# KKKSQJ/DeepLearning

Measured on NVIDIA H100. Metric: images/sec (ResNet-50 training step), higher is better.
Workload: dtype bf16

## Files before the change

deeplearning_b200/csrc/abi_conv.cu:

```cuda
#include <string.h>
#include "../../include/b200cls.h"
#include "conv_gemm.cuh"
#include "conv1x1_stream.cuh"
#include "conv_tap64.cuh"
#include "host_utils.h"
#include "wgrad_gemm.cuh"

using namespace b200;

namespace {

constexpr uint32_t kFwdDescLbo = 16, kFwdDescSbo = 1024;
constexpr uint32_t kWgDescLbo = 8192, kWgDescSbo = 1024, kWgDescKstep = 2048;

struct Box3 {
  int b1, b2, b3;
};

Box3 choose_box(long long d1, long long d2, long long d3, int P) {
  Box3 best{P, 1, 1};
  double best_cost = -1;
  for (int b1 = 1; b1 <= P; b1 <<= 1) {
    for (int b2 = 1; b1 * b2 <= P; b2 <<= 1) {
      const int b3 = P / (b1 * b2);
// ... 29 lines not shown
};

View make_view(const void* base, int B, int H, int W, int C, int s, int ph, int pw) {
  View v;
  v.base = static_cast<const char*>(base) + (static_cast<long long>(ph) * W + pw) * C * 2;
  v.dims[0] = C;
  v.dims[1] = (W - pw + s - 1) / s;
  v.dims[2] = (H - ph + s - 1) / s;
  v.dims[3] = B;
  v.strides[0] = 1;
  v.strides[1] = static_cast<uint64_t>(s) * C;
  v.strides[2] = static_cast<uint64_t>(s) * W * C;
  v.strides[3] = static_cast<uint64_t>(H) * W * C;
  return v;
}
View make_flat_view(const void* base, long long M, int C) {
  View v;
  v.base = base;
  v.dims[0] = C;
  v.dims[1] = M;
  v.dims[2] = 1;
  v.dims[3] = 1;
  v.strides[0] = 1;
  v.strides[1] = C;
  v.strides[2] = static_cast<uint64_t>(M) * C;
  v.strides[3] = static_cast<uint64_t>(M) * C;
  return v;
}
View act_view(const void* base, int B, int H, int W, int C, bool flat) {
  return flat ? make_flat_view(base, static_cast<long long>(B) * H * W, C) : make_view(base, B, H, W, C, 1, 0, 0);
}
int encode_view(CUtensorMap* m, const View& v, const Box3& bx) {
  uint32_t box[4] = {64, (uint32_t)bx.b1, (uint32_t)bx.b2, (uint32_t)bx.b3};
  if (v.dims[1] == 0 || v.dims[2] == 0 || v.dims[3] == 0) {
    set_error("empty activation view");
    return EINVAL_;
  }
  return encode_tmap_bf16(m, v.base, 4, v.dims, v.strides, box);
}

int encode_matrix(CUtensorMap* m, const void* base, long long cols, long long rows, int box_rows) {
  uint64_t dims[2] = {static_cast<uint64_t>(cols), static_cast<uint64_t>(rows)};
  uint64_t strides[2] = {1, static_cast<uint64_t>(cols)};
  uint32_t box[2] = {64, static_cast<uint32_t>(box_rows)};
  return encode_tmap_bf16(m, base, 2, dims, strides, box);
}

template <class Params>
int encode_taps(Params& p, CUtensorMap (&maps)[4], const void* x, int B, int H, int W, int C, int ksize, int stride,
                const Box3& bx) {
  int rc;
  if (stride == 1) {
    if ((rc = encode_view(&maps[0], act_view(x, B, H, W, C, ksize == 1), bx))) return rc;
    for (int i = 1; i < 4; ++i) maps[i] = maps[0];
  } else {
    for (int ph = 0; ph < 2; ++ph)
      for (int pw = 0; pw < 2; ++pw)
        if ((rc = encode_view(&maps[ph * 2 + pw], make_view(x, B, H, W, C, 2, ph, pw), bx))) return rc;
  }
  const int pad = pad_of(ksize);
  for (int kh = 0; kh < ksize; ++kh)
    for (int kw = 0; kw < ksize; ++kw) {
      const int t = kh * ksize + kw, dh = kh - pad, dw = kw - pad;
      const int ph = stride == 2 ? dh & 1 : 0, pw = stride == 2 ? dw & 1 : 0;
      p.tap_map[t] = static_cast<int8_t>(ph * 2 + pw);
      p.tap_o1[t] = static_cast<int8_t>((dw - pw) / stride);
      p.tap_o2[t] = static_cast<int8_t>((dh - ph) / stride);
    }
  return OK;
}

void quarter_box(const Box3& bx, Box3* qb, int (&o1)[4], int (&o2)[4], int (&o3)[4]) {
  for (int q = 0; q < 4; ++q) o1[q] = o2[q] = o3[q] = 0;
  if (bx.b3 >= 4) {
    *qb = Box3{bx.b1, bx.b2, bx.b3 / 4};
    for (int q = 0; q < 4; ++q) o3[q] = q * (bx.b3 / 4);
  } else if (bx.b3 == 2) {
    *qb = Box3{bx.b1, bx.b2 / 2, 1};
    if (bx.b2 >= 2) {
      for (int q = 0; q < 4; ++q) {
        o2[q] = (q & 1) * (bx.b2 / 2);
        o3[q] = q >> 1;
      }
    } else {
      *qb = Box3{bx.b1 / 2, 1, 1};
      for (int q = 0; q < 4; ++q) {
        o1[q] = (q & 1) * (bx.b1 / 2);
        o3[q] = q >> 1;
      }
    }
  } else if (bx.b2 >= 4) {
    *qb = Box3{bx.b1, bx.b2 / 4, 1};
    for (int q = 0; q < 4; ++q) o2[q] = q * (bx.b2 / 4);
  } else if (bx.b2 == 2) {
    *qb = Box3{bx.b1 / 2, 1, 1};
    for (int q = 0; q < 4; ++q) {
      o1[q] = (q & 1) * (bx.b1 / 2);
      o2[q] = q >> 1;
    }
  } else {
    *qb = Box3{bx.b1 / 4, 1, 1};
    for (int q = 0; q < 4; ++q) o1[q] = q * (bx.b1 / 4);
  }
}

int setup_output(ConvGemmParams& p, const View& dv, int N, int out_f32, const View* auxv) {
  const long long d1 = dv.dims[1], d2 = dv.dims[2], d3 = dv.dims[3];
  const Box3 bx = choose_box(d1, d2, d3, 128);
  p.box1 = bx.b1, p.box2 = bx.b2, p.box3 = bx.b3;
  p.dim1 = static_cast<int>(d1), p.dim2 = static_cast<int>(d2), p.dim3 = static_cast<int>(d3);
  p.tiles1 = static_cast<int>((d1 + bx.b1 - 1) / bx.b1);
  p.tiles2 = static_cast<int>((d2 + bx.b2 - 1) / bx.b2);
  p.tiles3 = static_cast<int>((d3 + bx.b3 - 1) / bx.b3);
  p.N = N;
  const int BN = N <= 64 ? 64 : 128;
  p.n_tiles = (N + BN - 1) / BN;
  Box3 qb;
  quarter_box(bx, &qb, p.qoff1, p.qoff2, p.qoff3);
  p.out_f32 = out_f32;
  if (dv.base != nullptr) {
    uint32_t box[4] = {out_f32 ? 32u : 64u, (uint32_t)qb.b1, (uint32_t)qb.b2, (uint32_t)qb.b3};
    int rc = out_f32 ? encode_tmap_f32(&p.d_map, dv.base, 4, dv.dims, dv.strides, box)
                     : encode_tmap_bf16(&p.d_map, dv.base, 4, dv.dims, dv.strides, box);
    if (rc) return rc;
  }
  p.has_aux_out = 0;
  if (auxv != nullptr) {
    uint32_t box[4] = {64u, (uint32_t)qb.b1, (uint32_t)qb.b2, (uint32_t)qb.b3};
    int rc = encode_tmap_bf16(&p.aux_map, auxv->base, 4, auxv->dims, auxv->strides, box);
    if (rc) return rc;
    p.has_aux_out = 1;
  }
  return OK;
}
Box3 box_of(const ConvGemmParams& p) { return Box3{p.box1, p.box2, p.box3}; }

bool bn_mask_complete(const b200_bn_mask_t* m) { return m->x_raw && m->scale && m->shift && m->stats; }
void set_bn_mask(ConvGemmParams& p, const b200_bn_mask_t* m, const View& dv) {
  p.mask_in = static_cast<const __nv_bfloat16*>(m->x_raw);
  p.ms1 = static_cast<long long>(dv.strides[1]);
  p.ms2 = static_cast<long long>(dv.strides[2]);
  p.ms3 = static_cast<long long>(dv.strides[3]);
  p.bn_scale = m->scale, p.bn_shift = m->shift, p.stats = m->stats;
}

int conv_grid(int tiles, int n_tiles, bool stats) {
  int grid = tiles < device_sm_count() ? tiles : device_sm_count();
  if (stats) grid = grid / n_tiles * n_tiles;
  return grid;
}

template <int BLOCK_N, int EPI>
int launch_conv_gemm_epi(const ConvGemmParams& q, int grid, cudaStream_t st) {
  using Cfg = ConvGemmCfg<BLOCK_N>;
  static bool configured = false;
  if (!configured) {
    B200_CHECK_CUDA(cudaFuncSetAttribute(conv_gemm_kernel<BLOCK_N, EPI>, cudaFuncAttributeMaxDynamicSharedMemorySize,
                                         Cfg::SMEM_BYTES));
    configured = true;
  }
  B200_CHECK_CUDA(launch_pdl(conv_gemm_kernel<BLOCK_N, EPI>, dim3(grid), dim3(Cfg::THREADS), Cfg::SMEM_BYTES, st, q));
  B200_LAUNCHED();
  return OK;
}

int epilogue_flags(const ConvGemmParams& p) {
  int f = 0;
  if (p.bias) f |= kEpiBias;
  if (p.colscale) f |= kEpiColscale;
  f |= (p.act & 3) << kEpiActShift;
  if (p.residual) f |= p.res_f32 ? kEpiResF32 : kEpiResBf16;
  if (p.has_aux_out) f |= kEpiAux;
  if (p.out_f32) f |= kEpiOutF32;
  if (p.out_direct) f |= kEpiDirect;
  if (p.stats) f |= kEpiStats;
  if (p.rowscale) f |= kEpiRowscale;
  if (p.affine) f = (f & ~(kEpiBias | kEpiColscale)) | kEpiAffine;
  if (p.mask_in) f |= p.bn_scale ? kEpiBnMask : kEpiMask;
  if (p.bn_scale) f &= ~kEpiStats;
  return f;
}

#define B200_EPI_LIST(X)                                                                                  \
  X(kEpiStats)                                              \
  X(0)                                                      \
  X(kEpiResBf16)                                            \
  X(kEpiBias)                                               \
  X(kEpiBias | kEpiResF32 | kEpiOutF32)                     \
  X(kEpiBias | kEpiColscale | kEpiResF32 | kEpiOutF32)      \
  X(kEpiBias | (2 << kEpiActShift) | kEpiAux)               \
  X(3 << kEpiActShift)                                      \
  X((3 << kEpiActShift) | kEpiStats)                        \
  X(kEpiOutF32)                                             \
  X(kEpiBias | kEpiOutF32)                                  \
  X(kEpiAffine | kEpiResBf16 | (1 << kEpiActShift))        \
  X(kEpiAffine | (1 << kEpiActShift))                      \
  X(kEpiAffine)                                            \
  X(kEpiMask | kEpiResBf16 | kEpiStats)                    \
  X(kEpiBnMask)                                            \
  X(kEpiBnMask | kEpiBias)

bool tap64_ok(const ConvGemmParams& p) {
  const int f = epilogue_flags(p);
  return p.N == 64 && p.n_tiles == 1 && p.k_per_tap == 64 && p.k_blocks_per_tap == 1 && !p.var_taps && !p.chan_window &&
         p.num_taps >= 2 && p.num_taps <= 9 && (f == 0 || f == kEpiStats) && p.dim1 % p.box1 == 0 && p.dim2 % p.box2 == 0 &&
         p.dim3 % p.box3 == 0;
}
template <bool kStats>
int launch_tap64(const ConvGemmParams& q, int grid, cudaStream_t st) {
  static bool configured = false;
  if (!configured) {
    B200_CHECK_CUDA(cudaFuncSetAttribute(conv_tap64_kernel<kStats>, cudaFuncAttributeMaxDynamicSharedMemorySize, kTap64SmemBytes));
    configured = true;
  }
  B200_CHECK_CUDA(launch_pdl(conv_tap64_kernel<kStats>, dim3(grid), dim3(384), kTap64SmemBytes, st, q));
  B200_LAUNCHED();
  return OK;
}

template <int BLOCK_N>
int launch_conv_gemm(const ConvGemmParams& p, cudaStream_t st) {
  const int tiles = p.tiles1 * p.tiles2 * p.tiles3 * p.n_tiles;
  const int grid = conv_grid(tiles, p.n_tiles, p.stats != nullptr);
  B200_REQUIRE(grid > 0, "conv_gemm: %d channel blocks exceed the SM count (BN statistics need grid %% n_tiles == 0)", p.n_tiles);
  ConvGemmParams q = p;
  q.desc_lbo = kFwdDescLbo;
  q.desc_sbo = kFwdDescSbo;
  if constexpr (BLOCK_N == 64) {
    if (tap64_ok(p)) return p.stats != nullptr ? launch_tap64<true>(q, grid, st) : launch_tap64<false>(q, grid, st);
  }
  switch (epilogue_flags(p)) {
#define B200_EPI_CASE(F) \
  case (F):              \
    return launch_conv_gemm_epi<BLOCK_N, (F)>(q, grid, st);
    B200_EPI_LIST(B200_EPI_CASE)
#undef B200_EPI_CASE
    default:
      return launch_conv_gemm_epi<BLOCK_N, kEpiGeneric>(q, grid, st);
  }
}


bool stream_ok(long long pixels, int K, int N) {
  return (K == 64 || K == 128 || K == 256) && N % 256 == 0 && pixels % 128 == 0 && pixels / 128 < (1LL << 30);
}
int stream_grid(long long pixels, int N) {
  const int n_tiles = N / 256;
  const long long items = pixels / 128 * n_tiles;
  int grid = items < device_sm_count() ? static_cast<int>(items) : device_sm_count();
  return grid / n_tiles * n_tiles;
}

template <int KB, int MODE>
int launch_stream(const StreamParams& q, int grid, cudaStream_t st) {
  using Cfg = StreamCfg<KB, MODE>;
  static bool configured = false;
  if (!configured) {
    B200_CHECK_CUDA(cudaFuncSetAttribute(conv1x1_stream_kernel<KB, MODE>, cudaFuncAttributeMaxDynamicSharedMemorySize,
                                         Cfg::SMEM_BYTES));
    configured = true;
  }
  B200_CHECK_CUDA(launch_pdl(conv1x1_stream_kernel<KB, MODE>, dim3(grid), dim3(Cfg::THREADS), Cfg::SMEM_BYTES, st, q));
  B200_LAUNCHED();
  return OK;
}

int run_stream(int mode, const void* a, const void* w, void* out, const void* res, const void* mask, const float* scale,
               const float* shift, float* stats, long long pixels, int K, int N, cudaStream_t st) {
  StreamParams q;
  memset(&q, 0, sizeof(q));
  int rc;
  if ((rc = encode_matrix(&q.a_map, a, K, pixels, 128))) return rc;
  if ((rc = encode_matrix(&q.b_map, w, K, N, 256))) return rc;
  if ((rc = encode_matrix(&q.out_map, out, N, pixels, 16))) return rc;
  if (res != nullptr && (rc = encode_matrix(&q.res_map, res, N, pixels, 16))) return rc;
  if (mask != nullptr && (rc = encode_matrix(&q.mask_map, mask, N, pixels, 16))) return rc;
  q.m_tiles = static_cast<int>(pixels / 128);
  q.n_tiles = N / 256;
  q.N = N;
  q.scale = scale, q.shift = shift, q.stats = stats;
  const int grid = stream_grid(pixels, N);
  if (mode == kStreamAffine)
    return K == 64 ? launch_stream<1, kStreamAffine>(q, grid, st)
                   : (K == 128 ? launch_stream<2, kStreamAffine>(q, grid, st) : launch_stream<4, kStreamAffine>(q, grid, st));
  if (mode == kStreamBnRelu)
    return K == 64 ? launch_stream<1, kStreamBnRelu>(q, grid, st)
                   : (K == 128 ? launch_stream<2, kStreamBnRelu>(q, grid, st) : launch_stream<4, kStreamBnRelu>(q, grid, st));
  return K == 64 ? launch_stream<1, kStreamMask>(q, grid, st)
                 : (K == 128 ? launch_stream<2, kStreamMask>(q, grid, st) : launch_stream<4, kStreamMask>(q, grid, st));
}

int dispatch_conv_gemm(ConvGemmParams& p, int N, cudaStream_t st) {
  if (N <= 64) return launch_conv_gemm<64>(p, st);
  return launch_conv_gemm<128>(p, st);
}
int block_n_for(int N) { return N <= 64 ? 64 : 128; }

template <int BLOCK_NG, bool kGrouped = false>
int launch_wgrad(const WgradParams& p, cudaStream_t st) {
  using Cfg = WgradCfg<BLOCK_NG>;
  static bool configured = false;
  if (!configured) {
    if constexpr (kGrouped) {
      B200_CHECK_CUDA(cudaFuncSetAttribute(wgrad_gemm_kernel<BLOCK_NG, false, true>,
                                           cudaFuncAttributeMaxDynamicSharedMemorySize, Cfg::SMEM_BYTES));
    } else {
      B200_CHECK_CUDA(cudaFuncSetAttribute(wgrad_gemm_kernel<BLOCK_NG, false>, cudaFuncAttributeMaxDynamicSharedMemorySize,
// ... 601 lines not shown
```

deeplearning_b200/csrc/conv_gemm.cuh:

```cuda
#pragma once
#include <cstdio>
#include "common.cuh"

namespace b200 {

constexpr int kMaxTaps = 16;

struct alignas(64) ConvGemmParams {
  CUtensorMap a_maps[4];
  CUtensorMap b_map;
  CUtensorMap d_map;
  CUtensorMap aux_map;
  int num_taps;
  int k_per_tap;
  int k_blocks_per_tap;
  int tiles1, tiles2, tiles3;
  int box1, box2, box3;
  int dim1, dim2, dim3;
  int qoff1[4], qoff2[4], qoff3[4];
  int n_tiles;
  int N;
  int8_t tap_map[kMaxTaps];
  int8_t tap_o1[kMaxTaps];
  int8_t tap_o2[kMaxTaps];
  int8_t tap_w[kMaxTaps];
  float* stats;
  const float* bias;
  const float* colscale;
  int act;
  int out_f32;
  int res_f32;
  int has_aux_out;
  const void* residual;
  long long rs1, rs2, rs3;
  const __nv_bfloat16* aux_in;
  long long as1, as2, as3;
  uint32_t desc_lbo, desc_sbo;
  float* out_direct;
  long long ld_out;
  const float* rowscale;
  int rows_per_sample;
  int var_taps;
  int kb_total;
  int16_t tap_kb[kMaxTaps];
  int32_t tap_k0[kMaxTaps];
  const __nv_bfloat16* mask_in;
  long long ms1, ms2, ms3;
  int affine;
  const float* bn_scale;
  const float* bn_shift;
  int chan_window;
};

template <int BLOCK_N>
struct ConvGemmCfg {
  static constexpr int BLOCK_M = 128;
  static constexpr int BLOCK_K = 64;
  static constexpr int A_BYTES = BLOCK_M * BLOCK_K * 2;
  static constexpr int B_BYTES = BLOCK_N * BLOCK_K * 2;
  static constexpr int STAGES = BLOCK_N == 128 ? 4 : 5;
  static constexpr int STAGE_BYTES = A_BYTES + B_BYTES;
  static constexpr int EPI_WARPS = 4;
  static constexpr int SLAB_BYTES = 32 * 128;
  static constexpr int STAGING_BYTES = EPI_WARPS * 2 * SLAB_BYTES;
  static constexpr int IMG_BYTES = BLOCK_M * BLOCK_N * 4;
  static constexpr int IMGS = BLOCK_N == 128 ? 1 : 2;
  static constexpr int BAR_BYTES = 256;
  static constexpr int SMEM_BYTES = STAGES * STAGE_BYTES + STAGING_BYTES + IMGS * IMG_BYTES + BAR_BYTES + 1024;
  static constexpr int THREADS = 512;
  static_assert(SMEM_BYTES <= 227 * 1024, "shared memory of one H100 block");
  static_assert(2 * STAGES + 2 * IMGS <= BAR_BYTES / 8, "mbarriers");
};

__device__ __forceinline__ void gelu_parts(float x, float& tail, float& e) {
  const float az = fabsf(x) * 0.70710678118654752f;
  float t;
  asm("rcp.approx.ftz.f32 %0, %1;" : "=f"(t) : "f"(fmaf(0.3275911f, az, 1.0f)));
  float poly = fmaf(1.061405429f, t, -1.453152027f);
  poly = fmaf(poly, t, 1.421413741f);
  poly = fmaf(poly, t, -0.284496736f);
  poly = fmaf(poly, t, 0.254829592f);
  asm("ex2.approx.ftz.f32 %0, %1;" : "=f"(e) : "f"(-1.4426950408889634f * az * az));
  tail = 0.5f * poly * t * e;
}
__device__ __forceinline__ float gelu_erf(float x) {
  float tail, e;
  gelu_parts(x, tail, e);
  return x * (x >= 0.f ? 1.0f - tail : tail);
}
__device__ __forceinline__ float gelu_erf_grad(float x) {
  float tail, e;
  gelu_parts(x, tail, e);
  const float cdf = x >= 0.f ? 1.0f - tail : tail;
  return fmaf(x * 0.3989422804014327f, e, cdf);
}

__device__ __forceinline__ void gelu_parts2(float x0, float x1, uint64_t& cdf, uint64_t& e) {
  const uint64_t az = f2_pack(fabsf(x0) * 0.70710678118654752f, fabsf(x1) * 0.70710678118654752f);
  float d0, d1, t0, t1, g0, g1, e0, e1, h0, h1;
  f2_unpack(f2_fma(f2_bcast(0.3275911f), az, f2_bcast(1.0f)), d0, d1);
  asm("rcp.approx.ftz.f32 %0, %1;" : "=f"(t0) : "f"(d0));
  asm("rcp.approx.ftz.f32 %0, %1;" : "=f"(t1) : "f"(d1));
  const uint64_t t = f2_pack(t0, t1);
  uint64_t poly = f2_fma(f2_bcast(1.061405429f), t, f2_bcast(-1.453152027f));
  poly = f2_fma(poly, t, f2_bcast(1.421413741f));
  poly = f2_fma(poly, t, f2_bcast(-0.284496736f));
  poly = f2_fma(poly, t, f2_bcast(0.254829592f));
  f2_unpack(f2_mul(f2_mul(az, az), f2_bcast(-1.4426950408889634f)), g0, g1);
  asm("ex2.approx.ftz.f32 %0, %1;" : "=f"(e0) : "f"(g0));
  asm("ex2.approx.ftz.f32 %0, %1;" : "=f"(e1) : "f"(g1));
  e = f2_pack(e0, e1);
  f2_unpack(f2_fma(f2_mul(f2_mul(poly, t), e), f2_bcast(-0.5f), f2_bcast(0.5f)), h0, h1);
  cdf = f2_add(f2_pack(copysignf(h0, x0), copysignf(h1, x1)), f2_bcast(0.5f));
}
__device__ __forceinline__ void gelu_erf2(float& x0, float& x1) {
  uint64_t cdf, e;
  gelu_parts2(x0, x1, cdf, e);
  f2_unpack(f2_mul(f2_pack(x0, x1), cdf), x0, x1);
}
__device__ __forceinline__ void gelu_erf_val_grad2(float& x0, float& x1, float& g0, float& g1) {
  uint64_t cdf, e;
  gelu_parts2(x0, x1, cdf, e);
  const uint64_t x = f2_pack(x0, x1);
  f2_unpack(f2_fma(f2_mul(x, f2_bcast(0.3989422804014327f)), e, cdf), g0, g1);
  f2_unpack(f2_mul(x, cdf), x0, x1);
}

#ifdef CONV_PROFILE
#define CPROF_DECL(N) long long cp_t[N] = {}; long long cp_0 = clock64(), cp_1;
#define CPROF_TICK(i) { cp_1 = clock64(); cp_t[i] += cp_1 - cp_0; cp_0 = cp_1; }
#else
#define CPROF_DECL(N)
#define CPROF_TICK(i)
#endif

template <int S>
__device__ __forceinline__ void butterfly_step(float (&px)[32], int lane) {
  const bool up = (lane & S) != 0;
#pragma unroll
  for (int i = 0; i < S; ++i) {
    const float send = up ? px[i] : px[i + S];
    const float keep = up ? px[i + S] : px[i];
    px[i] = keep + __shfl_xor_sync(0xffffffffu, send, S);
  }
}

constexpr int kEpiGeneric = -1;
constexpr int kEpiBias = 1, kEpiColscale = 2, kEpiActShift = 2 , kEpiResBf16 = 16, kEpiResF32 = 32,
              kEpiAux = 64, kEpiOutF32 = 128, kEpiDirect = 256, kEpiStats = 512,
              kEpiRowscale = 1024 ,
              kEpiAffine = 2048, kEpiMask = 4096, kEpiBnMask = 8192;

template <int BLOCK_N, int EPI = kEpiGeneric>
__global__ void __launch_bounds__(512, 1) conv_gemm_kernel(const __grid_constant__ ConvGemmParams p) {
  static_assert(BLOCK_N == 64 || BLOCK_N == 128, "64- or 128-column tiles");
  using Cfg = ConvGemmCfg<BLOCK_N>;
  constexpr int STAGES = Cfg::STAGES;
  constexpr int IMGS = Cfg::IMGS;
  extern __shared__ uint8_t smem_raw[];
  uint8_t* smem = reinterpret_cast<uint8_t*>((reinterpret_cast<uintptr_t>(smem_raw) + 1023) & ~uintptr_t(1023));
  uint8_t* stage_base = smem;
  uint8_t* staging = smem + STAGES * Cfg::STAGE_BYTES;
  uint8_t* img = staging + Cfg::STAGING_BYTES;
  uint64_t* bars = reinterpret_cast<uint64_t*>(img + IMGS * Cfg::IMG_BYTES);
  uint64_t* full_bar = bars;
  uint64_t* empty_bar = bars + STAGES;
  uint64_t* img_full = bars + 2 * STAGES;
  uint64_t* img_empty = bars + 2 * STAGES + IMGS;

  const int warp_idx = threadIdx.x >> 5;
  const int lane = threadIdx.x & 31;
  const int m_tiles = p.tiles1 * p.tiles2 * p.tiles3;
  const int num_tiles = m_tiles * p.n_tiles;
  const int num_kb = p.var_taps ? p.kb_total : p.num_taps * p.k_blocks_per_tap;

  if (warp_idx == 0 && lane == 0) {
    for (int i = 0; i < 4; ++i) tma_prefetch_desc(&p.a_maps[i]);
    tma_prefetch_desc(&p.b_map);
    tma_prefetch_desc(&p.d_map);
    for (int i = 0; i < STAGES; ++i) {
      mbar_init(&full_bar[i], 1);
      mbar_init(&empty_bar[i], 2);
    }
    for (int i = 0; i < IMGS; ++i) {
      mbar_init(&img_full[i], 8);
      mbar_init(&img_empty[i], Cfg::EPI_WARPS);
    }
    fence_mbar_init();
  }
  __syncthreads();
  pdl_wait();

  if (warp_idx < 4) {
    setmaxnreg_dec<40>();
    if (warp_idx == 0 && lane == 0) {
      int stage = 0;
      uint32_t phase = 0;
      CPROF_DECL(2)
      for (int tile = blockIdx.x; tile < num_tiles; tile += gridDim.x) {
        const int n_tile = tile % p.n_tiles;
        const int m_tile = tile / p.n_tiles;
        const int t1 = m_tile % p.tiles1;
        const int t2 = (m_tile / p.tiles1) % p.tiles2;
        const int t3 = m_tile / (p.tiles1 * p.tiles2);
        const int c1 = t1 * p.box1, c2 = t2 * p.box2, c3 = t3 * p.box3;
        int tap = 0, cb = 0;
        int kb_in_tap = p.var_taps ? p.tap_kb[0] : p.k_blocks_per_tap;
        for (int kb = 0; kb < num_kb; ++kb, ++cb) {
          if (cb == kb_in_tap) {
            cb = 0;
            ++tap;
            if (p.var_taps) kb_in_tap = p.tap_kb[tap];
          }
          const int wk = p.var_taps ? p.tap_k0[tap] + cb * 64 : p.tap_w[tap] * p.k_per_tap + cb * 64;
          CPROF_TICK(1)
          mbar_wait_backoff(&empty_bar[stage], phase ^ 1);
          CPROF_TICK(0)
          uint8_t* a_dst = stage_base + stage * Cfg::STAGE_BYTES;
          uint8_t* b_dst = a_dst + Cfg::A_BYTES;
          mbar_expect_tx(&full_bar[stage], Cfg::STAGE_BYTES);
          tma_load_4d(a_dst, &p.a_maps[p.tap_map[tap]], &full_bar[stage], p.chan_window ? n_tile * BLOCK_N : cb * 64, c1 + p.tap_o1[tap],
                      c2 + p.tap_o2[tap], c3);
          tma_load_2d(b_dst, &p.b_map, &full_bar[stage], wk, n_tile * BLOCK_N);
          if (++stage == STAGES) {
            stage = 0;
            phase ^= 1;
          }
        }
      }
#ifdef CONV_PROFILE
      if (blockIdx.x == 0) {
        const int nt = (num_tiles - 1) / gridDim.x + 1;
        printf("conv producer: wait_empty %lld issue %lld  (cycles/tile, %d tiles, %d k-blocks)\n", cp_t[0] / nt, cp_t[1] / nt, nt, num_kb);
      }
#endif
    }
  } else if (warp_idx < 12) {
    setmaxnreg_dec<112>();
    const int wg = (warp_idx - 4) >> 2;
    const uint64_t desc_a0 = make_smem_desc_sw128(smem_u32(stage_base) + wg * 8192, p.desc_lbo, p.desc_sbo);
    const uint64_t desc_b0 = make_smem_desc_sw128(smem_u32(stage_base) + Cfg::A_BYTES, p.desc_lbo, p.desc_sbo);
    int stage = 0;
    uint32_t phase = 0;
    int it = 0;
    CPROF_DECL(3)
    for (int tile = blockIdx.x; tile < num_tiles; tile += gridDim.x, ++it) {
      float acc[BLOCK_N / 2];
#pragma unroll
      for (int i = 0; i < BLOCK_N / 2; ++i) acc[i] = 0.f;
      int prev = -1;
      CPROF_TICK(2)
      for (int kb = 0; kb < num_kb; ++kb) {
        mbar_wait(&full_bar[stage], phase);
        wgmma_fence();
        const uint64_t soff = static_cast<uint64_t>(stage) * (Cfg::STAGE_BYTES >> 4);
        const uint64_t da = desc_a0 + soff, db = desc_b0 + soff;
#pragma unroll
        for (int k = 0; k < 4; ++k) Wgmma<BLOCK_N, 0, 0>::mma(acc, da + 2 * k, db + 2 * k, 1u);
        wgmma_commit();
        wgmma_wait<1>();
        if (prev >= 0 && (threadIdx.x & 127) == 0) mbar_arrive(&empty_bar[prev]);
        prev = stage;
        if (++stage == STAGES) {
          stage = 0;
          phase ^= 1;
        }
      }
      wgmma_wait<0>();
      wgmma_reg_fence(acc);
      if ((threadIdx.x & 127) == 0) mbar_arrive(&empty_bar[prev]);
      CPROF_TICK(0)
      const int b = IMGS == 1 ? 0 : it % IMGS;
      mbar_wait(&img_empty[b], ((it / IMGS) & 1) ^ 1);
      CPROF_TICK(1)
      acc_to_img<BLOCK_N>(acc, smem_u32(img + b * Cfg::IMG_BYTES), BLOCK_N, 64 * wg, 0);
      __syncwarp();
      if (lane == 0) mbar_arrive(&img_full[b]);
    }
#ifdef CONV_PROFILE
    if (blockIdx.x == 0 && lane == 0 && (warp_idx & 3) == 0) {
      const int nt = (num_tiles - 1) / gridDim.x + 1;
      printf("conv mma wg %d: main loop %lld wait img_empty %lld acc->img %lld  (cycles/tile)\n", wg, cp_t[0] / nt, cp_t[1] / nt,
             cp_t[2] / nt);
    }
#endif
  } else {
    setmaxnreg_inc<248>();
    const int q = warp_idx - 12;
    const int row = q * 32 + lane;
    const uint32_t stage_s = smem_u32(staging + q * 2 * Cfg::SLAB_BYTES);
    const uint32_t row_s = lane * 128;
    const uint32_t sw = (lane & 7) << 4;
    uint32_t stat_off[8];
#pragma unroll
    for (int m = 0; m < 8; ++m) stat_off[m] = m * 128 + ((((lane >> 2) ^ m) << 4) | ((lane & 3) << 2));
    constexpr bool G = EPI < 0;
    constexpr bool kAffine = !G && (EPI & kEpiAffine) != 0;
    constexpr bool kBnMask = !G && (EPI & kEpiBnMask) != 0;
    constexpr bool kMask = !G && (EPI & (kEpiMask | kEpiBnMask)) != 0;
    const int N = p.N;
    const float* const bias = (!kAffine && (G || (EPI & kEpiBias))) ? p.bias : nullptr;
    const float* const colscale = (!kAffine && (G || (EPI & kEpiColscale))) ? p.colscale : nullptr;
    const int act_bits = G ? p.act : ((EPI >> kEpiActShift) & 3);
    const int act = kAffine ? 0 : act_bits;
    const bool has_res = G ? (p.residual != nullptr) : ((EPI & (kEpiResBf16 | kEpiResF32)) != 0);
    const bool res_f32 = G ? (p.res_f32 != 0) : ((EPI & kEpiResF32) != 0);
    const bool has_aux = G ? (p.has_aux_out != 0) : ((EPI & kEpiAux) != 0);
    const bool out_f32 = G ? (p.out_f32 != 0) : ((EPI & kEpiOutF32) != 0);
    float* const out_direct = (G || (EPI & kEpiDirect)) ? p.out_direct : nullptr;
    float* const stats = (G || (EPI & (kEpiStats | kEpiBnMask))) ? p.stats : nullptr;
    const float* const rowscale = G ? p.rowscale : nullptr;
    const bool need_rowmap = has_res || act == 3 || kMask || out_direct != nullptr || rowscale != nullptr || p.dim1 % p.box1 != 0 ||
                             p.dim2 % p.box2 != 0 || p.dim3 % p.box3 != 0;
    const bool full_cols = (N % BLOCK_N) == 0;
    uint32_t store_counter = 0;
    const int unit_cols = out_f32 ? 32 : 64;
    const int units = BLOCK_N / unit_cols;
    const int nsub = out_f32 ? 1 : 2;
    constexpr int SLOTS = 2;
    uint64_t run_s[SLOTS], run_q[SLOTS];
    float run_x[SLOTS][2];
#pragma unroll
    for (int k = 0; k < SLOTS; ++k) run_s[k] = 0, run_q[k] = 0, run_x[k][0] = run_x[k][1] = 0.f;
    int it = 0;
    CPROF_DECL(2)
    for (int tile = blockIdx.x; tile < num_tiles; tile += gridDim.x, ++it) {
      const int b = IMGS == 1 ? 0 : it % IMGS;
      const uint32_t img_s = smem_u32(img + b * Cfg::IMG_BYTES);
      const int n_tile = tile % p.n_tiles;
      const int m_tile = tile / p.n_tiles;
      const int t1 = m_tile % p.tiles1;
      const int t2 = (m_tile / p.tiles1) % p.tiles2;
      const int t3 = m_tile / (p.tiles1 * p.tiles2);
      const int c1 = t1 * p.box1, c2 = t2 * p.box2, c3 = t3 * p.box3;
      int p1 = 0, p2 = 0, p3 = 0;
      bool row_ok = true;
      if (need_rowmap) {
        const int i1 = row % p.box1;
        const int i2 = (row / p.box1) % p.box2;
        const int i3 = row / (p.box1 * p.box2);
        p1 = c1 + i1, p2 = c2 + i2, p3 = c3 + i3;
        row_ok = (p1 < p.dim1) && (p2 < p.dim2) && (p3 < p.dim3);
      }
      const int s1 = c1 + p.qoff1[q], s2 = c2 + p.qoff2[q], s3 = c3 + p.qoff3[q];

      uint4 nx_b[4];
      float4 nx_f[8];
      uint4 nx_m[4];
      auto issue_pre = [&](int u, int h) {
        const int ncp = n_tile * BLOCK_N + u * unit_cols + h * 32;
        if (n_tile * BLOCK_N + u * unit_cols >= N || !row_ok) return;
        if (has_res) {
          const long long off = p3 * p.rs3 + p2 * p.rs2 + p1 * p.rs1 + ncp;
          if (res_f32) {
            const float4* rp = reinterpret_cast<const float4*>(static_cast<const float*>(p.residual) + off);
#pragma unroll
            for (int j = 0; j < 8; ++j)
              if (full_cols || ncp + j * 4 < N) nx_f[j] = __ldg(rp + j);
          } else {
            const uint4* rp = reinterpret_cast<const uint4*>(static_cast<const __nv_bfloat16*>(p.residual) + off);
#pragma unroll
            for (int j = 0; j < 4; ++j)
              if (full_cols || ncp + j * 8 < N) nx_b[j] = __ldg(rp + j);
          }
        }
        if (act == 3) {
          const uint4* ap = reinterpret_cast<const uint4*>(p.aux_in + p3 * p.as3 + p2 * p.as2 + p1 * p.as1 + ncp);
#pragma unroll
          for (int j = 0; j < 4; ++j)
            if (full_cols || ncp + j * 8 < N) nx_b[j] = __ldg(ap + j);
        }
        if constexpr (kMask) {
          const uint4* mp = reinterpret_cast<const uint4*>(p.mask_in + p3 * p.ms3 + p2 * p.ms2 + p1 * p.ms1 + ncp);
#pragma unroll
          for (int j = 0; j < 4; ++j)
            if (full_cols || ncp + j * 8 < N) nx_m[j] = __ldg(mp + j);
        }
      };
      if (has_res || act == 3 || kMask) issue_pre(0, 0);
      CPROF_TICK(1)
      mbar_wait(&img_full[b], (it / IMGS) & 1);
      CPROF_TICK(0)

#pragma unroll 1
      for (int u = 0; u < units; ++u) {
        const int n0 = n_tile * BLOCK_N + u * unit_cols;
        const bool chunk_live = n0 < N;
        const uint32_t buf_s = stage_s + (store_counter & 1) * Cfg::SLAB_BYTES;
        const uint32_t aux_s = stage_s + ((store_counter + 1) & 1) * Cfg::SLAB_BYTES;
        if (chunk_live && out_direct == nullptr) {
          if (lane == 0) {
            if (has_aux) tma_store_wait_read<0>(); else tma_store_wait_read<1>();
          }
          __syncwarp();
        }
#pragma unroll 1
        for (int h = 0; h < nsub; ++h) {
          uint32_t v[32];
          img_ld32(img_s, BLOCK_N, row, u * unit_cols + h * 32, v);
          if (u == units - 1 && h == nsub - 1) {
            __syncwarp();
            if (lane == 0) mbar_arrive(&img_empty[b]);
          }
          uint4 pre_b[4];
          float4 pre_f[8];
          uint4 pre_m[4];
          if (has_res || act == 3 || kMask) {
#pragma unroll
            for (int j = 0; j < 4; ++j) pre_b[j] = nx_b[j];
#pragma unroll
            for (int j = 0; j < 8; ++j) pre_f[j] = nx_f[j];
            if constexpr (kMask) {
#pragma unroll
              for (int j = 0; j < 4; ++j) pre_m[j] = nx_m[j];
            }
            if (h + 1 < nsub)
              issue_pre(u, h + 1);
            else if (u + 1 < units)
              issue_pre(u + 1, 0);
          }
          if (!chunk_live) continue;
          const int nc = n0 + h * 32;
          float f[32];
#pragma unroll
          for (int j = 0; j < 32; ++j) f[j] = __uint_as_float(v[j]);
          if constexpr (kAffine) {
#pragma unroll
            for (int j = 0; j < 8; ++j) {
              const float4 s4 = __ldg(reinterpret_cast<const float4*>(p.colscale + nc) + j);
              const float4 b4 = __ldg(reinterpret_cast<const float4*>(p.bias + nc) + j);
              f2_unpack(f2_fma(f2_pack(f[j * 4 + 0], f[j * 4 + 1]), f2_pack(s4.x, s4.y), f2_pack(b4.x, b4.y)), f[j * 4 + 0], f[j * 4 + 1]);
              f2_unpack(f2_fma(f2_pack(f[j * 4 + 2], f[j * 4 + 3]), f2_pack(s4.z, s4.w), f2_pack(b4.z, b4.w)), f[j * 4 + 2], f[j * 4 + 3]);
            }
          }
          if (bias != nullptr) {
            if (full_cols) {
#pragma unroll
              for (int j = 0; j < 8; ++j) {
                const float4 b4 = __ldg(reinterpret_cast<const float4*>(bias + nc) + j);
                f2_unpack(f2_add(f2_pack(f[j * 4 + 0], f[j * 4 + 1]), f2_pack(b4.x, b4.y)), f[j * 4 + 0], f[j * 4 + 1]);
                f2_unpack(f2_add(f2_pack(f[j * 4 + 2], f[j * 4 + 3]), f2_pack(b4.z, b4.w)), f[j * 4 + 2], f[j * 4 + 3]);
              }
            } else {
#pragma unroll
              for (int j = 0; j < 32; ++j) f[j] += (nc + j < N) ? __ldg(bias + nc + j) : 0.0f;
            }
          }
          if (has_aux) {
            const uint32_t z = row_ok ? 0xffffffffu : 0u;
            if (act == 2) {
#pragma unroll
              for (int j = 0; j < 4; ++j) {
                float g[8];
#pragma unroll
                for (int i = 0; i < 8; i += 2) gelu_erf_val_grad2(f[j * 8 + i], f[j * 8 + i + 1], g[i], g[i + 1]);
                sts128(aux_s + row_s + ((((h * 4 + j) << 4)) ^ sw), pack_bf16x2(g[0], g[1]) & z, pack_bf16x2(g[2], g[3]) & z,
                       pack_bf16x2(g[4], g[5]) & z, pack_bf16x2(g[6], g[7]) & z);
              }
            } else {
#pragma unroll
              for (int j = 0; j < 4; ++j)
                sts128(aux_s + row_s + ((((h * 4 + j) << 4)) ^ sw), pack_bf16x2(f[j * 8 + 0], f[j * 8 + 1]) & z,
                       pack_bf16x2(f[j * 8 + 2], f[j * 8 + 3]) & z, pack_bf16x2(f[j * 8 + 4], f[j * 8 + 5]) & z,
                       pack_bf16x2(f[j * 8 + 6], f[j * 8 + 7]) & z);
            }
          }
          if (act == 1) {
#pragma unroll
            for (int j = 0; j < 32; ++j) f[j] = fmaxf(f[j], 0.0f);
          } else if (act == 2) {
            if (!has_aux) {
#pragma unroll
              for (int j = 0; j < 32; j += 2) gelu_erf2(f[j], f[j + 1]);
            }
          } else if (act == 3 && row_ok) {
#pragma unroll
            for (int j = 0; j < 4; ++j) {
              if (full_cols || nc + j * 8 < N) {
                float a[8];
                unpack8(pre_b[j], a);
#pragma unroll
                for (int i = 0; i < 8; i += 2)
                  f2_unpack(f2_mul(f2_pack(f[j * 8 + i], f[j * 8 + i + 1]), f2_pack(a[i], a[i + 1])), f[j * 8 + i],
                            f[j * 8 + i + 1]);
              }
            }
          }
          if (colscale != nullptr) {
#pragma unroll
            for (int j = 0; j < 32; ++j) f[j] *= (full_cols || nc + j < N) ? __ldg(colscale + nc + j) : 0.0f;
          }
          if (rowscale != nullptr && row_ok) {
            const long long pix = (static_cast<long long>(p3) * p.dim2 + p2) * p.dim1 + p1;
            const float rs = __ldg(rowscale + pix / p.rows_per_sample);
#pragma unroll
            for (int j = 0; j < 32; ++j) f[j] *= rs;
          }
          if (has_res && row_ok) {
            if (res_f32) {
#pragma unroll
              for (int j = 0; j < 8; ++j) {
                if (full_cols || nc + j * 4 < N) {
                  const float4 r = pre_f[j];
                  f2_unpack(f2_add(f2_pack(f[j * 4 + 0], f[j * 4 + 1]), f2_pack(r.x, r.y)), f[j * 4 + 0], f[j * 4 + 1]);
                  f2_unpack(f2_add(f2_pack(f[j * 4 + 2], f[j * 4 + 3]), f2_pack(r.z, r.w)), f[j * 4 + 2], f[j * 4 + 3]);
                }
              }
            } else {
#pragma unroll
              for (int j = 0; j < 4; ++j) {
                if (full_cols || nc + j * 8 < N) {
                  float r[8];
                  unpack8(pre_b[j], r);
#pragma unroll
                  for (int i = 0; i < 8; i += 2)
                    f2_unpack(f2_add(f2_pack(f[j * 8 + i], f[j * 8 + i + 1]), f2_pack(r[i], r[i + 1])), f[j * 8 + i],
                              f[j * 8 + i + 1]);
                }
              }
            }
          }
          if constexpr (kAffine) {
            if (act_bits == 1) {
#pragma unroll
              for (int j = 0; j < 32; ++j) f[j] = fmaxf(f[j], 0.0f);
            }
          }
          if constexpr (kBnMask) {
            float px[32];
            if (row_ok) {
#pragma unroll
              for (int j = 0; j < 4; ++j) {
                float x8[8];
                unpack8(pre_m[j], x8);
#pragma unroll
                for (int i = 0; i < 8; ++i) px[j * 8 + i] = x8[i];
              }
#pragma unroll
              for (int j = 0; j < 8; ++j) {
                const float4 s4 = __ldg(reinterpret_cast<const float4*>(p.bn_scale + nc) + j);
                const float4 b4 = __ldg(reinterpret_cast<const float4*>(p.bn_shift + nc) + j);
                const float sc4[4] = {s4.x, s4.y, s4.z, s4.w}, sh4[4] = {b4.x, b4.y, b4.z, b4.w};
#pragma unroll
                for (int i = 0; i < 4; ++i) {
                  const float fm =
                      fmaf(px[j * 4 + i], sc4[i], sh4[i]) > 0.f ? __bfloat162float(__float2bfloat16_rn(f[j * 4 + i])) : 0.f;
                  f[j * 4 + i] = fm;
                  px[j * 4 + i] *= fm;
                }
              }
            } else {
#pragma unroll
              for (int j = 0; j < 32; ++j) px[j] = 0.f;
            }
            butterfly_step<16>(px, lane);
            butterfly_step<8>(px, lane);
            butterfly_step<4>(px, lane);
            butterfly_step<2>(px, lane);
            butterfly_step<1>(px, lane);
            const int slot = units == 1 ? (it & 1) : u;
#pragma unroll
            for (int k = 0; k < SLOTS; ++k) {
              if (k == slot) {
                run_x[k][0] += h == 0 ? px[0] : 0.f;
                run_x[k][1] += h == 0 ? 0.f : px[0];
              }
            }
          } else if constexpr (kMask) {
            if (row_ok) {
#pragma unroll
              for (int j = 0; j < 4; ++j) {
                const uint32_t w[4] = {pre_m[j].x, pre_m[j].y, pre_m[j].z, pre_m[j].w};
#pragma unroll
                for (int i = 0; i < 4; ++i) {
                  if ((w[i] & 0x7fffu) == 0u) f[j * 8 + 2 * i] = 0.f;
                  if ((w[i] & 0x7fff0000u) == 0u) f[j * 8 + 2 * i + 1] = 0.f;
                }
              }
            }
          }
          if (out_direct != nullptr) {
            if (row_ok) {
              const long long pix = (static_cast<long long>(p3) * p.dim2 + p2) * p.dim1 + p1;
              float* op = out_direct + pix * p.ld_out + nc;
#pragma unroll
              for (int j = 0; j < 32; ++j)
                if (nc + j < N) op[j] = f[j];
            }
            continue;
          }
          if (!row_ok) {
#pragma unroll
            for (int j = 0; j < 32; ++j) f[j] = 0.f;
          }
          if (out_f32) {
#pragma unroll
            for (int j = 0; j < 8; ++j)
              sts128(buf_s + row_s + ((j << 4) ^ sw), __float_as_uint(f[j * 4 + 0]), __float_as_uint(f[j * 4 + 1]),
                     __float_as_uint(f[j * 4 + 2]), __float_as_uint(f[j * 4 + 3]));
          } else {
#pragma unroll
            for (int j = 0; j < 4; ++j)
              sts128(buf_s + row_s + (((h * 4 + j) << 4) ^ sw), pack_bf16x2(f[j * 8 + 0], f[j * 8 + 1]),
                     pack_bf16x2(f[j * 8 + 2], f[j * 8 + 3]), pack_bf16x2(f[j * 8 + 4], f[j * 8 + 5]),
                     pack_bf16x2(f[j * 8 + 6], f[j * 8 + 7]));
          }
        }
        if (!chunk_live || out_direct != nullptr) continue;
        __syncwarp();
        if (stats != nullptr) {
          uint64_t a_s = 0, a_q = 0;
#pragma unroll
          for (int r = 0; r < 32; ++r) {
            const uint32_t w = lds32(buf_s + (r >> 3) * 1024 + stat_off[r & 7]);
            const uint64_t x2 = f2_pack(bf16_lo(w), bf16_hi(w));
            a_s = f2_add(a_s, x2);
            a_q = f2_fma(x2, x2, a_q);
          }
          const int slot = units == 1 ? (it & 1) : u;
#pragma unroll
          for (int k = 0; k < SLOTS; ++k) {
            if (k == slot) {
              run_s[k] = f2_add(run_s[k], a_s);
              run_q[k] = f2_add(run_q[k], a_q);
            }
          }
        }
        fence_proxy_async_smem();
        __syncwarp();
        if (lane == 0) {
          asm volatile("cp.async.bulk.tensor.4d.global.shared::cta.bulk_group [%0, {%2, %3, %4, %5}], [%1];" ::"l"(
                           reinterpret_cast<uint64_t>(&p.d_map)),
                       "r"(buf_s), "r"(n0), "r"(s1), "r"(s2), "r"(s3)
                       : "memory");
          tma_store_commit();
          if (has_aux) {
            asm volatile("cp.async.bulk.tensor.4d.global.shared::cta.bulk_group [%0, {%2, %3, %4, %5}], [%1];" ::"l"(
                             reinterpret_cast<uint64_t>(&p.aux_map)),
                         "r"(aux_s), "r"(n0), "r"(s1), "r"(s2), "r"(s3)
                         : "memory");
            tma_store_commit();
          }
        }
        store_counter += has_aux ? 2 : 1;
      }
    }
#ifdef CONV_PROFILE
    if (blockIdx.x == 0 && lane == 0 && q == 0) {
      const int nt = (num_tiles - 1) / gridDim.x + 1;
      printf("conv epilogue: wait img_full %lld drain %lld  (cycles/tile)\n", cp_t[0] / nt, cp_t[1] / nt);
    }
#endif
    if (stats != nullptr) {
      const int cta = static_cast<int>(blockIdx.x);
      const int n_tile = cta % p.n_tiles;
      const int grp = cta / p.n_tiles;
#pragma unroll
      for (int k = 0; k < SLOTS; ++k) {
        const int srow = units == 1 ? (grp * 4 + q) * 2 + k : grp * 4 + q;
        const int col = n_tile * BLOCK_N + (units == 1 ? 0 : k * unit_cols) + 2 * lane;
        if (col < N) {
          float s_lo, s_hi, q_lo, q_hi;
          f2_unpack(run_s[k], s_lo, s_hi);
          f2_unpack(run_q[k], q_lo, q_hi);
          float* sp = stats + static_cast<long long>(srow) * 2 * N + col;
          *reinterpret_cast<float2*>(sp) = make_float2(s_lo, s_hi);
          if constexpr (kBnMask) {
            sp += N - lane;
            sp[0] = run_x[k][0];
            sp[32] = run_x[k][1];
          } else {
            *reinterpret_cast<float2*>(sp + N) = make_float2(q_lo, q_hi);
          }
        }
      }
    }
    if (lane == 0) tma_store_wait_all<0>();
  }
}

}
```

Measured before the change: 8800.

## Add second epilogue warpgroup for BLOCK_N=64 and BN-mask conv GEMM kernels

Makes the conv GEMM config depend on the epilogue variant and adds a second epilogue warpgroup for 64-column tiles and BN-mask epilogues. The two groups either alternate tiles or split the columns of a single accumulator image. Register budgets per role are rebalanced with setmaxnreg, and stage counts drop to fit staging memory. The BN-mask path now keeps scale/shift in lanes and shuffles them, moves the product reduction after the store, and recomputes stats offsets to save registers. The aim is to stop the epilogue from bottlenecking the MMA pipeline, at the cost of fewer pipeline stages and tighter register limits per role.

```diff
diff --git a/deeplearning_b200/csrc/abi_conv.cu b/deeplearning_b200/csrc/abi_conv.cu
--- a/deeplearning_b200/csrc/abi_conv.cu
+++ b/deeplearning_b200/csrc/abi_conv.cu
@@ -205,7 +205,7 @@
 
 template <int BLOCK_N, int EPI>
 int launch_conv_gemm_epi(const ConvGemmParams& q, int grid, cudaStream_t st) {
-  using Cfg = ConvGemmCfg<BLOCK_N>;
+  using Cfg = ConvGemmCfg<BLOCK_N, EPI>;
   static bool configured = false;
   if (!configured) {
     B200_CHECK_CUDA(cudaFuncSetAttribute(conv_gemm_kernel<BLOCK_N, EPI>, cudaFuncAttributeMaxDynamicSharedMemorySize,
diff --git a/deeplearning_b200/csrc/conv_gemm.cuh b/deeplearning_b200/csrc/conv_gemm.cuh
--- a/deeplearning_b200/csrc/conv_gemm.cuh
+++ b/deeplearning_b200/csrc/conv_gemm.cuh
@@ -52,26 +52,6 @@
   int chan_window;
 };
 
-template <int BLOCK_N>
-struct ConvGemmCfg {
-  static constexpr int BLOCK_M = 128;
-  static constexpr int BLOCK_K = 64;
-  static constexpr int A_BYTES = BLOCK_M * BLOCK_K * 2;
-  static constexpr int B_BYTES = BLOCK_N * BLOCK_K * 2;
-  static constexpr int STAGES = BLOCK_N == 128 ? 4 : 5;
-  static constexpr int STAGE_BYTES = A_BYTES + B_BYTES;
-  static constexpr int EPI_WARPS = 4;
-  static constexpr int SLAB_BYTES = 32 * 128;
-  static constexpr int STAGING_BYTES = EPI_WARPS * 2 * SLAB_BYTES;
-  static constexpr int IMG_BYTES = BLOCK_M * BLOCK_N * 4;
-  static constexpr int IMGS = BLOCK_N == 128 ? 1 : 2;
-  static constexpr int BAR_BYTES = 256;
-  static constexpr int SMEM_BYTES = STAGES * STAGE_BYTES + STAGING_BYTES + IMGS * IMG_BYTES + BAR_BYTES + 1024;
-  static constexpr int THREADS = 512;
-  static_assert(SMEM_BYTES <= 227 * 1024, "shared memory of one H100 block");
-  static_assert(2 * STAGES + 2 * IMGS <= BAR_BYTES / 8, "mbarriers");
-};
-
 __device__ __forceinline__ void gelu_parts(float x, float& tail, float& e) {
   const float az = fabsf(x) * 0.70710678118654752f;
   float t;
@@ -145,16 +125,48 @@
   }
 }
 
+__device__ __forceinline__ float bf16_at(const uint4 (&m)[4], int k) {
+  const uint4 q = m[k >> 3];
+  const uint32_t w = (k & 6) == 0 ? q.x : (k & 6) == 2 ? q.y : (k & 6) == 4 ? q.z : q.w;
+  return (k & 1) ? bf16_hi(w) : bf16_lo(w);
+}
+
 constexpr int kEpiGeneric = -1;
 constexpr int kEpiBias = 1, kEpiColscale = 2, kEpiActShift = 2 , kEpiResBf16 = 16, kEpiResF32 = 32,
               kEpiAux = 64, kEpiOutF32 = 128, kEpiDirect = 256, kEpiStats = 512,
               kEpiRowscale = 1024 ,
               kEpiAffine = 2048, kEpiMask = 4096, kEpiBnMask = 8192;
 
+template <int BLOCK_N, int EPI>
+struct ConvGemmCfg {
+  static constexpr int BLOCK_M = 128;
+  static constexpr int BLOCK_K = 64;
+  static constexpr int A_BYTES = BLOCK_M * BLOCK_K * 2;
+  static constexpr int B_BYTES = BLOCK_N * BLOCK_K * 2;
+  static constexpr int EPI_WGS = BLOCK_N == 64 || (EPI >= 0 && (EPI & kEpiBnMask) != 0) ? 2 : 1;
+  static constexpr int STAGES = BLOCK_N == 128 && EPI_WGS == 2 ? 3 : 4;
+  static constexpr int STAGE_BYTES = A_BYTES + B_BYTES;
+  static constexpr int EPI_WARPS = 4 * EPI_WGS;
+  static constexpr int SLAB_BYTES = 32 * 128;
+  static constexpr int STAGING_BYTES = EPI_WARPS * 2 * SLAB_BYTES;
+  static constexpr int IMG_BYTES = BLOCK_M * BLOCK_N * 4;
+  static constexpr int IMGS = BLOCK_N == 128 ? 1 : 2;
+  static constexpr int BAR_BYTES = 256;
+  static constexpr int SMEM_BYTES = STAGES * STAGE_BYTES + STAGING_BYTES + IMGS * IMG_BYTES + BAR_BYTES + 1024;
+  static constexpr int THREADS = 128 * (3 + EPI_WGS);
+  static constexpr int LAUNCH_REGS = 65536 / THREADS / 8 * 8;
+  static constexpr int PRODUCER_REGS = EPI_WGS == 2 ? 24 : 40;
+  static constexpr int MMA_REGS = EPI_WGS == 1 ? 112 : (BLOCK_N == 128 ? 96 : 64);
+  static constexpr int EPI_REGS = EPI_WGS == 1 ? 248 : (BLOCK_N == 128 ? 128 : 160);
+  static_assert(PRODUCER_REGS + 2 * MMA_REGS + EPI_WGS * EPI_REGS <= (3 + EPI_WGS) * LAUNCH_REGS, "register file of one SM");
+  static_assert(SMEM_BYTES <= 227 * 1024, "shared memory of one H100 block");
+  static_assert(2 * STAGES + 2 * IMGS <= BAR_BYTES / 8, "mbarriers");
+};
+
 template <int BLOCK_N, int EPI = kEpiGeneric>
-__global__ void __launch_bounds__(512, 1) conv_gemm_kernel(const __grid_constant__ ConvGemmParams p) {
+__global__ void __launch_bounds__(ConvGemmCfg<BLOCK_N, EPI>::THREADS, 1) conv_gemm_kernel(const __grid_constant__ ConvGemmParams p) {
   static_assert(BLOCK_N == 64 || BLOCK_N == 128, "64- or 128-column tiles");
-  using Cfg = ConvGemmCfg<BLOCK_N>;
+  using Cfg = ConvGemmCfg<BLOCK_N, EPI>;
   constexpr int STAGES = Cfg::STAGES;
   constexpr int IMGS = Cfg::IMGS;
   extern __shared__ uint8_t smem_raw[];
@@ -167,6 +179,7 @@
   uint64_t* empty_bar = bars + STAGES;
   uint64_t* img_full = bars + 2 * STAGES;
   uint64_t* img_empty = bars + 2 * STAGES + IMGS;
+  constexpr bool kSplitCols = Cfg::EPI_WGS == 2 && IMGS == 1;
 
   const int warp_idx = threadIdx.x >> 5;
   const int lane = threadIdx.x & 31;
@@ -184,7 +197,7 @@
     }
     for (int i = 0; i < IMGS; ++i) {
       mbar_init(&img_full[i], 8);
-      mbar_init(&img_empty[i], Cfg::EPI_WARPS);
+      mbar_init(&img_empty[i], kSplitCols ? 8 : 4);
     }
     fence_mbar_init();
   }
@@ -192,7 +205,7 @@
   pdl_wait();
 
   if (warp_idx < 4) {
-    setmaxnreg_dec<40>();
+    setmaxnreg_dec<Cfg::PRODUCER_REGS>();
     if (warp_idx == 0 && lane == 0) {
       int stage = 0;
       uint32_t phase = 0;
@@ -236,7 +249,7 @@
 #endif
     }
   } else if (warp_idx < 12) {
-    setmaxnreg_dec<112>();
+    setmaxnreg_dec<Cfg::MMA_REGS>();
     const int wg = (warp_idx - 4) >> 2;
     const uint64_t desc_a0 = make_smem_desc_sw128(smem_u32(stage_base) + wg * 8192, p.desc_lbo, p.desc_sbo);
     const uint64_t desc_b0 = make_smem_desc_sw128(smem_u32(stage_base) + Cfg::A_BYTES, p.desc_lbo, p.desc_sbo);
@@ -285,15 +298,13 @@
     }
 #endif
   } else {
-    setmaxnreg_inc<248>();
-    const int q = warp_idx - 12;
+    setmaxnreg_inc<Cfg::EPI_REGS>();
+    const int ew = Cfg::EPI_WGS == 1 ? 0 : (warp_idx - 12) >> 2;
+    const int q = warp_idx & 3;
     const int row = q * 32 + lane;
-    const uint32_t stage_s = smem_u32(staging + q * 2 * Cfg::SLAB_BYTES);
+    const uint32_t stage_s = smem_u32(staging + (ew * 4 + q) * 2 * Cfg::SLAB_BYTES);
     const uint32_t row_s = lane * 128;
     const uint32_t sw = (lane & 7) << 4;
-    uint32_t stat_off[8];
-#pragma unroll
-    for (int m = 0; m < 8; ++m) stat_off[m] = m * 128 + ((((lane >> 2) ^ m) << 4) | ((lane & 3) << 2));
     constexpr bool G = EPI < 0;
     constexpr bool kAffine = !G && (EPI & kEpiAffine) != 0;
     constexpr bool kBnMask = !G && (EPI & kEpiBnMask) != 0;
@@ -317,14 +328,16 @@
     const int unit_cols = out_f32 ? 32 : 64;
     const int units = BLOCK_N / unit_cols;
     const int nsub = out_f32 ? 1 : 2;
-    constexpr int SLOTS = 2;
+    const int u_begin = kSplitCols ? ew * units / 2 : 0, u_end = kSplitCols ? (ew + 1) * units / 2 : units;
+    const int tile_wgs = kSplitCols ? 1 : Cfg::EPI_WGS;
+    constexpr int SLOTS = Cfg::EPI_WGS == 2 ? 1 : 2;
     uint64_t run_s[SLOTS], run_q[SLOTS];
     float run_x[SLOTS][2];
 #pragma unroll
     for (int k = 0; k < SLOTS; ++k) run_s[k] = 0, run_q[k] = 0, run_x[k][0] = run_x[k][1] = 0.f;
-    int it = 0;
     CPROF_DECL(2)
-    for (int tile = blockIdx.x; tile < num_tiles; tile += gridDim.x, ++it) {
+    for (int tile = blockIdx.x + (kSplitCols ? 0 : ew) * gridDim.x, it = kSplitCols ? 0 : ew; tile < num_tiles;
+         tile += tile_wgs * gridDim.x, it += tile_wgs) {
       const int b = IMGS == 1 ? 0 : it % IMGS;
       const uint32_t img_s = smem_u32(img + b * Cfg::IMG_BYTES);
       const int n_tile = tile % p.n_tiles;
@@ -377,13 +390,13 @@
             if (full_cols || ncp + j * 8 < N) nx_m[j] = __ldg(mp + j);
         }
       };
-      if (has_res || act == 3 || kMask) issue_pre(0, 0);
+      if (has_res || act == 3 || kMask) issue_pre(u_begin, 0);
       CPROF_TICK(1)
       mbar_wait(&img_full[b], (it / IMGS) & 1);
       CPROF_TICK(0)
 
 #pragma unroll 1
-      for (int u = 0; u < units; ++u) {
+      for (int u = u_begin; u < u_end; ++u) {
         const int n0 = n_tile * BLOCK_N + u * unit_cols;
         const bool chunk_live = n0 < N;
         const uint32_t buf_s = stage_s + (store_counter & 1) * Cfg::SLAB_BYTES;
@@ -398,7 +411,7 @@
         for (int h = 0; h < nsub; ++h) {
           uint32_t v[32];
           img_ld32(img_s, BLOCK_N, row, u * unit_cols + h * 32, v);
-          if (u == units - 1 && h == nsub - 1) {
+          if (u == u_end - 1 && h == nsub - 1) {
             __syncwarp();
             if (lane == 0) mbar_arrive(&img_empty[b]);
           }
@@ -416,7 +429,7 @@
             }
             if (h + 1 < nsub)
               issue_pre(u, h + 1);
-            else if (u + 1 < units)
+            else if (u + 1 < u_end)
               issue_pre(u + 1, 0);
           }
           if (!chunk_live) continue;
@@ -527,38 +540,82 @@
             }
           }
           if constexpr (kBnMask) {
-            float px[32];
-            if (row_ok) {
-#pragma unroll
-              for (int j = 0; j < 4; ++j) {
-                float x8[8];
-                unpack8(pre_m[j], x8);
-#pragma unroll
-                for (int i = 0; i < 8; ++i) px[j * 8 + i] = x8[i];
-              }
+            const float sc_l = kSplitCols ? __ldg(p.bn_scale + nc + lane) : 0.f;
+            const float sh_l = kSplitCols ? __ldg(p.bn_shift + nc + lane) : 0.f;
+            if (kSplitCols || row_ok) {
 #pragma unroll
               for (int j = 0; j < 8; ++j) {
-                const float4 s4 = __ldg(reinterpret_cast<const float4*>(p.bn_scale + nc) + j);
-                const float4 b4 = __ldg(reinterpret_cast<const float4*>(p.bn_shift + nc) + j);
-                const float sc4[4] = {s4.x, s4.y, s4.z, s4.w}, sh4[4] = {b4.x, b4.y, b4.z, b4.w};
+                float sc4[4], sh4[4];
+                if constexpr (kSplitCols) {
+#pragma unroll
+                  for (int i = 0; i < 4; ++i) {
+                    sc4[i] = __shfl_sync(0xffffffffu, sc_l, j * 4 + i);
+                    sh4[i] = __shfl_sync(0xffffffffu, sh_l, j * 4 + i);
+                  }
+                } else {
+                  const float4 s4 = __ldg(reinterpret_cast<const float4*>(p.bn_scale + nc) + j);
+                  const float4 b4 = __ldg(reinterpret_cast<const float4*>(p.bn_shift + nc) + j);
+                  sc4[0] = s4.x, sc4[1] = s4.y, sc4[2] = s4.z, sc4[3] = s4.w;
+                  sh4[0] = b4.x, sh4[1] = b4.y, sh4[2] = b4.z, sh4[3] = b4.w;
+                }
 #pragma unroll
                 for (int i = 0; i < 4; ++i) {
-                  const float fm =
-                      fmaf(px[j * 4 + i], sc4[i], sh4[i]) > 0.f ? __bfloat162float(__float2bfloat16_rn(f[j * 4 + i])) : 0.f;
-                  f[j * 4 + i] = fm;
-                  px[j * 4 + i] *= fm;
+                  if (!kSplitCols || row_ok)
+                    f[j * 4 + i] = fmaf(bf16_at(pre_m, j * 4 + i), sc4[i], sh4[i]) > 0.f
+                                       ? __bfloat162float(__float2bfloat16_rn(f[j * 4 + i]))
+                                       : 0.f;
                 }
               }
-            } else {
-#pragma unroll
-              for (int j = 0; j < 32; ++j) px[j] = 0.f;
-            }
+            }
+          } else if constexpr (kMask) {
+            if (row_ok) {
+#pragma unroll
+              for (int j = 0; j < 4; ++j) {
+                const uint32_t w[4] = {pre_m[j].x, pre_m[j].y, pre_m[j].z, pre_m[j].w};
+#pragma unroll
+                for (int i = 0; i < 4; ++i) {
+                  if ((w[i] & 0x7fffu) == 0u) f[j * 8 + 2 * i] = 0.f;
+                  if ((w[i] & 0x7fff0000u) == 0u) f[j * 8 + 2 * i + 1] = 0.f;
+                }
+              }
+            }
+          }
+          if (out_direct != nullptr) {
+            if (row_ok) {
+              const long long pix = (static_cast<long long>(p3) * p.dim2 + p2) * p.dim1 + p1;
+              float* op = out_direct + pix * p.ld_out + nc;
+#pragma unroll
+              for (int j = 0; j < 32; ++j)
+                if (nc + j < N) op[j] = f[j];
+            }
+            continue;
+          }
+          if (!row_ok) {
+#pragma unroll
+            for (int j = 0; j < 32; ++j) f[j] = 0.f;
+          }
+          if (out_f32) {
+#pragma unroll
+            for (int j = 0; j < 8; ++j)
+              sts128(buf_s + row_s + ((j << 4) ^ sw), __float_as_uint(f[j * 4 + 0]), __float_as_uint(f[j * 4 + 1]),
+                     __float_as_uint(f[j * 4 + 2]), __float_as_uint(f[j * 4 + 3]));
+          } else {
+#pragma unroll
+            for (int j = 0; j < 4; ++j)
+              sts128(buf_s + row_s + (((h * 4 + j) << 4) ^ sw), pack_bf16x2(f[j * 8 + 0], f[j * 8 + 1]),
+                     pack_bf16x2(f[j * 8 + 2], f[j * 8 + 3]), pack_bf16x2(f[j * 8 + 4], f[j * 8 + 5]),
+                     pack_bf16x2(f[j * 8 + 6], f[j * 8 + 7]));
+          }
+          if constexpr (kBnMask) {
+            float px[32];
+#pragma unroll
+            for (int k = 0; k < 32; ++k) px[k] = row_ok ? bf16_at(pre_m, k) * f[k] : 0.f;
             butterfly_step<16>(px, lane);
             butterfly_step<8>(px, lane);
             butterfly_step<4>(px, lane);
             butterfly_step<2>(px, lane);
             butterfly_step<1>(px, lane);
-            const int slot = units == 1 ? (it & 1) : u;
+            const int slot = Cfg::EPI_WGS == 2 ? 0 : (units == 1 ? (it & 1) : u);
 #pragma unroll
             for (int k = 0; k < SLOTS; ++k) {
               if (k == slot) {
@@ -566,44 +623,6 @@
                 run_x[k][1] += h == 0 ? 0.f : px[0];
               }
             }
-          } else if constexpr (kMask) {
-            if (row_ok) {
-#pragma unroll
-              for (int j = 0; j < 4; ++j) {
-                const uint32_t w[4] = {pre_m[j].x, pre_m[j].y, pre_m[j].z, pre_m[j].w};
-#pragma unroll
-                for (int i = 0; i < 4; ++i) {
-                  if ((w[i] & 0x7fffu) == 0u) f[j * 8 + 2 * i] = 0.f;
-                  if ((w[i] & 0x7fff0000u) == 0u) f[j * 8 + 2 * i + 1] = 0.f;
-                }
-              }
-            }
-          }
-          if (out_direct != nullptr) {
-            if (row_ok) {
-              const long long pix = (static_cast<long long>(p3) * p.dim2 + p2) * p.dim1 + p1;
-              float* op = out_direct + pix * p.ld_out + nc;
-#pragma unroll
-              for (int j = 0; j < 32; ++j)
-                if (nc + j < N) op[j] = f[j];
-            }
-            continue;
-          }
-          if (!row_ok) {
-#pragma unroll
-            for (int j = 0; j < 32; ++j) f[j] = 0.f;
-          }
-          if (out_f32) {
-#pragma unroll
-            for (int j = 0; j < 8; ++j)
-              sts128(buf_s + row_s + ((j << 4) ^ sw), __float_as_uint(f[j * 4 + 0]), __float_as_uint(f[j * 4 + 1]),
-                     __float_as_uint(f[j * 4 + 2]), __float_as_uint(f[j * 4 + 3]));
-          } else {
-#pragma unroll
-            for (int j = 0; j < 4; ++j)
-              sts128(buf_s + row_s + (((h * 4 + j) << 4) ^ sw), pack_bf16x2(f[j * 8 + 0], f[j * 8 + 1]),
-                     pack_bf16x2(f[j * 8 + 2], f[j * 8 + 3]), pack_bf16x2(f[j * 8 + 4], f[j * 8 + 5]),
-                     pack_bf16x2(f[j * 8 + 6], f[j * 8 + 7]));
           }
         }
         if (!chunk_live || out_direct != nullptr) continue;
@@ -612,12 +631,12 @@
           uint64_t a_s = 0, a_q = 0;
 #pragma unroll
           for (int r = 0; r < 32; ++r) {
-            const uint32_t w = lds32(buf_s + (r >> 3) * 1024 + stat_off[r & 7]);
+            const uint32_t w = lds32(buf_s + r * 128 + ((((lane >> 2) ^ (r & 7)) << 4) | ((lane & 3) << 2)));
             const uint64_t x2 = f2_pack(bf16_lo(w), bf16_hi(w));
             a_s = f2_add(a_s, x2);
             a_q = f2_fma(x2, x2, a_q);
           }
-          const int slot = units == 1 ? (it & 1) : u;
+          const int slot = Cfg::EPI_WGS == 2 ? 0 : (units == 1 ? (it & 1) : u);
 #pragma unroll
           for (int k = 0; k < SLOTS; ++k) {
             if (k == slot) {
@@ -647,8 +666,8 @@
     }
 #ifdef CONV_PROFILE
     if (blockIdx.x == 0 && lane == 0 && q == 0) {
-      const int nt = (num_tiles - 1) / gridDim.x + 1;
-      printf("conv epilogue: wait img_full %lld drain %lld  (cycles/tile)\n", cp_t[0] / nt, cp_t[1] / nt);
+      const int nt = (num_tiles - 1) / (tile_wgs * gridDim.x) + 1;
+      printf("conv epilogue wg %d: wait img_full %lld drain %lld  (cycles/tile)\n", ew, cp_t[0] / nt, cp_t[1] / nt);
     }
 #endif
     if (stats != nullptr) {
@@ -657,8 +676,9 @@
       const int grp = cta / p.n_tiles;
 #pragma unroll
       for (int k = 0; k < SLOTS; ++k) {
-        const int srow = units == 1 ? (grp * 4 + q) * 2 + k : grp * 4 + q;
-        const int col = n_tile * BLOCK_N + (units == 1 ? 0 : k * unit_cols) + 2 * lane;
+        const int ks = Cfg::EPI_WGS == 2 ? ew : k;
+        const int srow = units == 1 ? (grp * 4 + q) * 2 + ks : grp * 4 + q;
+        const int col = n_tile * BLOCK_N + (units == 1 ? 0 : ks * unit_cols) + 2 * lane;
         if (col < N) {
           float s_lo, s_hi, q_lo, q_hi;
           f2_unpack(run_s[k], s_lo, s_hi);
```

New measurement: 8979, median of 6. 2.0% higher.
